# AlwinEsch/pvr.rtl.radiofm

Hardware: AMD Instinct MI355X
Metric: IQ MS/s demodulated (whole node) + achieved HBM GB/s on FIR stage (higher is better)
Workload: dtype f32

## Files before the change

### pvr.rtl.radiofm_amd/csrc/fmd_batch.hip

```cpp
#include "../../include/fmd.h"

#include <hip/hip_runtime.h>
#include <hip/hip_ext.h>

#include <algorithm>
#include <chrono>
#include <cmath>
#include <cstdio>
#include <cstdlib>
#include <cstring>
#include <deque>
#include <functional>
#include <map>
#include <memory>
#include <mutex>
#include <string>
#include <utility>
#include <vector>

#include "fmd_design.hpp"
#include "fmd_groups.hpp"
#include "fmd_kernels.hip.h"
#include "fmd_receiver.hpp"

// ... 19 lines not shown
enum Stage
{
  ST_IF_FIR = 0,
  ST_DEMOD_SERIAL,
  ST_RDS_HALFBAND,
  ST_RDS_LPF,
  ST_RDS_SERIAL,
  ST_RESAMPLE,
  ST_AUDIO_LPF,
  ST_AUDIO_TAIL,
  ST_ROLL,
  ST_COUNT
};
const char* kStageNames[ST_COUNT] = {"if_fir",      "demod_serial", "rds_halfband",
                                     "rds_lpf",     "rds_serial",   "resample",
                                     "audio_lpf",   "audio_tail",   "history_roll"};

template <typename T, bool HOST>
struct Buf
{
  T* p = nullptr;
  size_t n = 0;
  Buf() = default;
  Buf(Buf&& o) noexcept : p(std::exchange(o.p, nullptr)), n(std::exchange(o.n, 0)) {}
  ~Buf() { release(); }
  int alloc(size_t count, unsigned host_flags = hipHostMallocDefault)
  {
    release();
    const size_t bytes = std::max<size_t>(count, 1) * sizeof(T);
    void* v = nullptr;
    if ((HOST ? hipHostMalloc(&v, bytes, host_flags) : hipMalloc(&v, bytes)) != hipSuccess)
      return -1;
    p = static_cast<T*>(v);
    if (HOST)
      std::memset(v, 0, bytes);
    else if (hipMemset(v, 0, bytes) != hipSuccess)
    {
      release();
      return -1;
    }
    n = count;
    return 0;
  }
  void release()
  {
    if (p)
      (void)(HOST ? hipHostFree(p) : hipFree(p));
    p = nullptr;
    n = 0;
  }
};
template <typename T>
using DevBuf = Buf<T, false>;
template <typename T>
using HostBuf = Buf<T, true>;

struct Event
{
  hipEvent_t e = nullptr;
  Event() = default;
  Event(Event&& o) noexcept : e(std::exchange(o.e, nullptr)) {}
  ~Event() { release(); }
  hipError_t create(unsigned flags = hipEventDisableTiming)
  {
    release();
    return hipEventCreateWithFlags(&e, flags);
  }
  void release()
  {
    if (e)
      (void)hipEventDestroy(e);
    e = nullptr;
  }
  operator hipEvent_t() const { return e; }
};

template <typename... P, typename... A>
void launch(void (*kern)(P...), dim3 grid, dim3 block, unsigned lds, hipStream_t s, hipEvent_t ev_start,
            hipEvent_t ev_stop, A... args)
{
  static_assert(sizeof...(P) == sizeof...(A), "kernel argument count");
  if (ev_start)
    hipExtLaunchKernelGGL(kern, grid, block, lds, s, ev_start, ev_stop, 0u, static_cast<P>(args)...);
  else
    hipLaunchKernelGGL(kern, grid, block, lds, s, static_cast<P>(args)...);
}

}

struct fmd_batch
{
  fmd::Params params;
  fmd::Design des;
  unsigned C = 0, CP = 0;
  int device = 0;
  fmd_callbacks cb{};
  void* user = nullptr;
  std::vector<int> shifts;

  unsigned if_pos = 0;
  unsigned lut_idx = 0;
  float rs_pos = 0.0f;
  unsigned rds_lpf_g = 0;
  unsigned mf_g = 0;
  unsigned alpf_g = 0;
  int hist_sel = 0;
  uint32_t call_index = 0;

  unsigned min_samples = 0;
  int streams_sharing = 0;
  unsigned cpc = 1;
  unsigned Mmax = 0, Mstride = 0, Amax = 0, Rmax = 0;
  std::vector<unsigned> hb_nmax;
  unsigned lastM = 0, lastA = 0, lastR = 0;

  DevBuf<float2> lut, hist[2], demod[2], br[2], mix[2], rdsraw[2], rlpf[2], rs[2], alp[2];
  std::vector<DevBuf<float2>> hbbuf;
  DevBuf<float> if_coeff, rs_coeff, rds_lpf_taps, mf_taps2, audio_taps, ktab;
  DevBuf<float> rpll, rmf, tap_sync;
  DevBuf<double> sctab, sctab256;
  DevBuf<int> pidx;
  static constexpr unsigned kBrFront = 32;
  float2* brp(int q) const { return br[q].p + size_t(kBrFront) * CP; }
  unsigned rs_margin = 0, rs_row = 0;
  int rsr_R = 0, rsr_NW = 0;
  unsigned rsr_nbr = 0, rsr_nbm = 0;
  int rsr_rb = 0;
  DevBuf<float> rsr_tab;
  DevBuf<int> rsr_head, rsr_steps;
  int rsr_mode = -1;
  int n_cus = 256;
  struct HbfPlan
  {
    unsigned n_in = 0, S = 0;
    DevBuf<fmd::HbStep> steps;
    DevBuf<int> seg_first;
  };
  std::vector<std::unique_ptr<HbfPlan>> hbf_plans;
  DevBuf<float2> hbf_tail1, hbf_tail2;
  int hbf_mode = -1;
  static constexpr unsigned kOscH = 64;
  DevBuf<fmd::HbOsc> osc_tab[4];
  HostBuf<fmd::HbOsc> h_osc;
  Event osc_ev[8];
  bool osc_ev_used[8] = {};
  size_t h_osc_stride = 0;
  float osc_re = 1.0f, osc_im = 0.0f;
  bool osc_on = false;
  int dbg_nomix = 1;
  int dbg_fir_nt = 0;
  int dbg_serial_claim = 0;
  int dbg_hb4 = 1, dbg_ring4 = 1;
  int dbg_fir_ro = 2;
  int dbg_lpf_late = -1;
  double host_ms[4] = {0, 0, 0, 0};
  unsigned host_calls = 0;
  DevBuf<long long> serial_probe;
  int dbg_stage_mask = 63;
  DevBuf<float> fstate;
  DevBuf<int> istate;
  DevBuf<uint16_t> r_data;
  static constexpr int NSLOT = 8;
  static_assert(NSLOT == 8, "osc_ev / osc_ev_used above");
  DevBuf<fmd::RdsGroupRec> queue[NSLOT];
  DevBuf<unsigned> queue_counts;
  unsigned* qcount(int q) const { return queue_counts.p + q; }
  uint32_t drained_call[NSLOT] = {};
  HostBuf<unsigned> h_counts;
  HostBuf<fmd::RdsGroupRec> h_recs;
  unsigned queue_cap = 0;
  Event ev_drained[NSLOT];
  bool drained_pending[NSLOT] = {};
  static constexpr unsigned kExportCursors = 16;
  DevBuf<unsigned> export_cursor;
  unsigned export_seq = 0;
  fmd::ChannelState st{};
  std::vector<fmd::HbCoef> hbcoef;
  fmd::HbChainTaps hb_taps{};

  DevBuf<float> h_iq, h_audio;
  DevBuf<float> h_mpx;
  int dbg_mpx_timing = 0;
  Event mpx_ev[8][2];
  bool mpx_ev_used[8] = {};
  DevBuf<unsigned long long> pcm_clip;

  struct SelTable
  {
    DevBuf<int> d;
    HostBuf<int> h;
    Event read;
    hipStream_t stream = nullptr;
    bool used = false;
  };
  struct Selection
  {
    bool on = false;
    unsigned n_total = 0;
    std::vector<unsigned> list;
    std::vector<int2> ent;
    bool dirty = false;
    std::vector<std::unique_ptr<SelTable>> pool;
    int cur = -1;
  };
  Selection sel_audio, sel_mpx;
  bool decoder_owned = false;

  std::vector<std::unique_ptr<fmd::GroupDecoder>> gdec;

  int profiling = 0;
  int write_taps = 0;

  int concurrency = 1;
  hipStream_t s_fir = nullptr, s_ser = nullptr, s_post = nullptr, s_rds = nullptr, s_lpf = nullptr;
  struct LightJob
  {
    unsigned R = 0, A = 0, mf_g = 0, alpf_g = 0;
    unsigned rds_lpf_g = 0;
    const unsigned* org = nullptr;
    int q = 0, es = 0, sq = 0;
    bool events = true;
    bool lpf_here = false;
    int audio_after = -1;
    bool status_after_rds = false;
    hipEvent_t prev_aud = nullptr;
    uint32_t call_index = 0;
    void* d_audio = nullptr;
    int pcm = 0;
    size_t audio_stride = 0;
    hipEvent_t tl0 = nullptr, tl1 = nullptr;
    Selection* asel = nullptr;
  };
  std::vector<std::unique_ptr<fmd_batch>> subs;
  std::vector<unsigned> sub_ch0;
  bool owns_streams = true;
  hipEvent_t vheavy[2] = {nullptr, nullptr};
  hipEvent_t sched_prev2 = nullptr;
  bool split_post = false;
  bool serial_exclusive = false;
  enum { EV_IN, EV_FIR, EV_INDONE, EV_SER, EV_AUD, EV_RDS, EV_HEAVY, EV_RDSH, EV_ALP, EV_DEC, EV_ROLL, EV_N };
  Event cev[NSLOT][EV_N];
  uint32_t slot_call[NSLOT] = {};
  std::vector<Event> ev;
  unsigned prof_calls = 0;

  HostBuf<unsigned> h_err;
  bool failed = false;
  std::string fail_msg;
  unsigned spin_limit = 1u << 20;
  bool if_dry_run = false;
  HostBuf<unsigned> h_status;
  DevBuf<unsigned> d_status;
  unsigned host_seq = 0;

  fmd_params cparams{};
  std::unique_ptr<fmd_batch> twin;
  DevBuf<float2> twin_iq;
  DevBuf<float> twin_audio;
  std::mutex log_mu;
  std::vector<std::vector<std::pair<uint32_t, int>>> shift_log;
  std::vector<uint32_t> gdec_epoch;
  struct Edit
  {
    unsigned ch;
    int shift;
    bool reset;
    int imp = -1;
  };
  std::vector<Edit> edits;
  bool edits_pending = false;
  fmd::RestartTable restart_tab{};
  int restart_group[fmd::kRestartMaxRegions] = {};
  int restart_skip = -1;
  unsigned restart_rows_cap = 0;
  HostBuf<int2> h_edits;
  HostBuf<float2> h_rows;
  DevBuf<int2> d_edits;
  DevBuf<float2> d_rows;
  Event edit_ev[NSLOT];
  bool edit_ev_used[NSLOT] = {};
  Event edit_done;
  unsigned restart_seq = 0;
  DevBuf<unsigned> org;
  bool origins_live = false;
  int dbg_reset_keep_phase = 0;

  unsigned n_cap = 0;
  bool map_on = false, map_dirty = false;
  int capture_walk = 1;
  std::vector<unsigned> cmap;
  DevBuf<uint2> d_walk;
  HostBuf<uint2> h_walk;
  Event walk_ev[NSLOT];
  bool walk_ev_used[NSLOT] = {};

  fmd::StateTable state_tab{};
  int state_group[fmd::kStateMaxRegions] = {};
  size_t state_bytes = 0;
  int state_skip = -1;
  struct PendingImport
  {
    int slot = 0;
    unsigned n_cols = 0, n_rows = 0;
    size_t rows_at = 0, payload_at = 0, bytes = 0;
    bool origins_live = false;
    std::vector<fmd::StateEdit> list;
// ... 1366 lines not shown
}

int fmd_batch_process_device_u8(fmd_batch* b, const uint8_t* d_iq_u8, size_t iq_channel_stride,
                                unsigned samples, float* d_audio, size_t audio_channel_stride,
                                unsigned* out_floats, void* stream)
{
  return fmd_batch_process_device_fmt(b, d_iq_u8, FMD_IQ_U8, iq_channel_stride, samples, d_audio,
                                      audio_channel_stride, out_floats, stream);
}

static bool slot_eligible(const fmd_batch* b, int q, int lag)
{
  return b->slot_call[q] != 0 && b->slot_call[q] + uint32_t(lag) <= b->call_index;
}

static int wait_impl(fmd_batch* b, int lag, void* stream_, bool take_lost)
{
  if (!b || lag < 0 || lag > 4)
    return fail(FMD_ERR_ARG, "fmd_batch_wait: bad argument (lag must be 0..4)");
  hipStream_t stream = static_cast<hipStream_t>(stream_);
  HIPCHK(hipSetDevice(b->device));
  if (is_shell(b))
  {
    for (auto& sb : b->subs)
    {
      const int rc = wait_impl(sb.get(), lag, stream_, false);
      if (rc < 0)
        return check_device_errors(b);
    }
    if (int rc = check_device_errors(b))
      return rc;
    return take_lost ? take_lost_groups(b) : FMD_OK;
  }
  auto wait_if_pending = [&](hipEvent_t e) {
    if (hipEventQuery(e) == hipSuccess)
      return hipSuccess;
    (void)hipGetLastError();
    return hipStreamWaitEvent(stream, e, 0);
  };
  for (int q = 0; q < fmd_batch::NSLOT; q++)
    if (slot_eligible(b, q, lag))
    {
      HIPCHK(wait_if_pending(b->cev[q][fmd_batch::EV_AUD]));
      HIPCHK(wait_if_pending(b->cev[q][fmd_batch::EV_RDS]));
      HIPCHK(wait_if_pending(b->cev[q][fmd_batch::EV_INDONE]));
      HIPCHK(wait_if_pending(b->cev[q][fmd_batch::EV_ROLL]));
    }
  if (int rc = check_device_errors(b))
    return rc;
  return take_lost ? take_lost_groups(b) : FMD_OK;
}

int fmd_batch_wait_lagged(fmd_batch* b, int lag, void* stream_)
{
  return wait_impl(b, lag, stream_, true);
}

int fmd_batch_take_rds_lost(fmd_batch* b)
{
  if (!b)
    return fail(FMD_ERR_ARG, "null batch");
  return take_lost_groups(b) == FMD_WARN_RDS_LOST ? 1 : 0;
}

int fmd_batch_debug_set_spin_limit(fmd_batch* b, unsigned limit)
{
  if (!b)
    return fail(FMD_ERR_ARG, "null batch");
  b->spin_limit = limit;
  b->st.spin_limit = limit;
  for (auto& sb : b->subs)
    fmd_batch_debug_set_spin_limit(sb.get(), limit);
  return FMD_OK;
}

int fmd_batch_debug_restart_skip(fmd_batch* b, int region)
{
  if (!b)
    return fail(FMD_ERR_ARG, "null batch");
  if (region < -1 || region >= kRestartRegionCount)
  {
    std::string names;
    for (const char* r : kRestartRegions)
      names += std::string(names.empty() ? "" : ", ") + r;
    return fail(FMD_ERR_ARG, "fmd_batch_debug_restart_skip: -1 or the index of a region (" + names + ")");
  }
  b->restart_skip = region;
  for (auto& sb : b->subs)
    sb->restart_skip = region;
  return FMD_OK;
}

int fmd_batch_debug_reset_keep_ring_phase(fmd_batch* b, int on)
{
  if (!b)
    return fail(FMD_ERR_ARG, "null batch");
  b->dbg_reset_keep_phase = on != 0;
  for (auto& sb : b->subs)
    sb->dbg_reset_keep_phase = on != 0;
  return FMD_OK;
}

int fmd_batch_debug_host_ms(fmd_batch* b, float out[4])
{
  if (!b || !out)
    return fail(FMD_ERR_ARG, "null argument");
  const unsigned n = b->host_calls;
  for (int i = 0; i < 4; i++)
  {
    out[i] = n ? float(b->host_ms[i] / n) : 0.0f;
    b->host_ms[i] = 0.0;
  }
  b->host_calls = 0;
  return int(n);
}

int fmd_batch_debug_set(fmd_batch* b, const char* key, int value)
{
  if (!b || !key)
    return fail(FMD_ERR_ARG, "null argument");
  const std::string k(key);
  HIPCHK(hipSetDevice(b->device));
  HIPCHK(hipDeviceSynchronize());
  if (is_shell(b))
  {
    for (auto& sb : b->subs)
      if (int rc = fmd_batch_debug_set(sb.get(), key, value))
        return rc;
    return FMD_OK;
  }
  if (k == "resampler")
  {
    if (value > 0 && b->rsr_R == 0)
      return fail(FMD_ERR_ARG, "fmd_batch_debug_set: no form of k_resample_ring fits this geometry");
    b->rsr_mode = value < 0 ? -1 : (value ? 1 : 0);
  }
  else if (k == "fir_nt")
    b->dbg_fir_nt = std::max(0, value);
  else if (k == "serial_claim")
    b->dbg_serial_claim = value != 0;
  else if (k == "serial_exclusive")
    b->serial_exclusive = value != 0;
  else if (k == "split_post")
    b->split_post = value != 0;
  else if (k == "hb4")
    b->dbg_hb4 = value != 0;
  else if (k == "ring4")
    b->dbg_ring4 = value != 0;
  else if (k == "lpf_late")
    b->dbg_lpf_late = value < 0 ? -1 : std::min(value, 2);
  else if (k == "stage_mask")
    b->dbg_stage_mask = value & 63;
  else if (k == "fir_ro")
    b->dbg_fir_ro = (value == 2 || value == 3) ? value : 1;
  else if (k == "serial_probe")
  {
    HIPCHK(hipSetDevice(b->device));
    HIPCHK(hipDeviceSynchronize());
    b->serial_probe.release();
    if (value && b->serial_probe.alloc(size_t(8) * 3 * (b->CP / 64)))
      return fail(FMD_ERR_DEVICE, "serial probe allocation failed");
  }
  else if (k == "halfband_chain")
  {
    b->hbf_mode = value < 0 ? -1 : (value ? 1 : 0);
    if (value > 0 && b->call_index == 0 && b->h_osc.p && b->des.hb.size() == 3 &&
        b->des.hb[0].len - 1 <= int(fmd_batch::kOscH))
      b->osc_on = true;
  }
  else if (k == "nomix")
    b->dbg_nomix = value != 0;
  else if (k == "rsr_form")
  {
    bool ok = false;
    for (int f = std::max(0, std::min(2, value)); f < 3 && !ok; f++)
      ok = rsr_configure(b, f);
  }
  else
    return fail(FMD_ERR_ARG, "fmd_batch_debug_set: unknown key '" + k + "'");
  return FMD_OK;
}

int fmd_batch_enable_retune(fmd_batch* b)
{
  if (!b)
    return fail(FMD_ERR_ARG, "fmd_batch_enable_retune: null batch");
  if (b->twin)
    return FMD_OK;
  if (b->call_index != 0)
    return fail(FMD_ERR_STATE, "fmd_batch_enable_retune: only before the batch's first call");
  HIPCHK(hipSetDevice(b->device));
  fmd_batch* tw = nullptr;
  const int zero_shift = 0;
  if (int rc = create_one(&b->cparams, 1, &zero_shift, b->device, nullptr, nullptr, b, &tw))
    return rc;
  std::unique_ptr<fmd_batch> twin(tw);
  twin->concurrency = 2;
  if (b->twin_iq.alloc(FMD_MAX_BLOCK) || b->twin_audio.alloc(fmd_batch_max_audio_floats(tw, FMD_MAX_BLOCK)))
    return fail(FMD_ERR_DEVICE, "fmd_batch_enable_retune: device allocation failed");
  if (is_shell(b))
  {
    for (auto& sb : b->subs)
      if (int rc = build_restart_table(sb.get(), tw))
        return rc;
  }
  else if (int rc = build_restart_table(b, tw))
    return rc;
  HIPCHK(hipDeviceSynchronize());
  {
    std::lock_guard<std::mutex> lk(b->log_mu);
    b->shift_log.resize(b->C);
  }
  b->gdec_epoch.resize(b->C, 0u);
  b->twin = std::move(twin);
  return FMD_OK;
}

int fmd_batch_retune_channels(fmd_batch* b, const unsigned* channels, const int* shifts, unsigned n)
{
  if (!b || !channels || !shifts)
    return fail(FMD_ERR_ARG, "fmd_batch_retune_channels: null argument");
  if (b->failed)
    return fail(FMD_ERR_ARG, "fmd_batch_retune_channels: the batch has failed (fmd_batch_reset clears it)");
  if (!b->twin)
    return fail(FMD_ERR_STATE, "fmd_batch_retune_channels: retuning is not enabled (fmd_batch_enable_retune)");
  if (int rc = check_channel_list(b, channels, nullptr, n, "fmd_batch_retune_channels"))
    return rc;
  const uint32_t k = b->call_index + 1;
  std::lock_guard<std::mutex> lk(b->log_mu);
  for (unsigned i = 0; i < n; i++)
  {
    unsigned lc = 0;
    fmd_batch* ob = owner_of(b, channels[i], &lc);
    ob->edits.push_back(fmd_batch::Edit{lc, shifts[i], false});
    drop_gdec_import(b, channels[i], k);
    auto& log = b->shift_log[channels[i]];
    if (!log.empty() && log.back().first == k)
      log.back().second = shifts[i];
    else
      log.emplace_back(k, shifts[i]);
  }
  b->edits_pending = true;
  return FMD_OK;
}

int fmd_batch_reset_channels(fmd_batch* b, const unsigned* channels, unsigned n)
{
  if (!b || !channels)
    return fail(FMD_ERR_ARG, "fmd_batch_reset_channels: null argument");
  if (b->failed)
    return fail(FMD_ERR_ARG, "fmd_batch_reset_channels: the batch has failed (fmd_batch_reset clears it)");
  std::vector<unsigned> seen(channels, channels + n);
  std::sort(seen.begin(), seen.end());
  if (n && seen.back() >= b->C)
    return fail(FMD_ERR_ARG, "fmd_batch_reset_channels: channel " + std::to_string(seen.back()) + " out of range");
  if (std::adjacent_find(seen.begin(), seen.end()) != seen.end())
    return fail(FMD_ERR_ARG, "fmd_batch_reset_channels: a channel is listed twice");
  if (n == 0)
    return FMD_OK;
  const uint32_t k = b->call_index + 1;
  std::lock_guard<std::mutex> lk(b->log_mu);
  if (b->shift_log.empty())
  {
    b->shift_log.resize(b->C);
    b->gdec_epoch.assign(b->C, 0u);
  }
  for (unsigned i = 0; i < n; i++)
  {
    unsigned lc = 0;
    fmd_batch* ob = owner_of(b, channels[i], &lc);
    ob->edits.push_back(fmd_batch::Edit{lc, 0, true});
    drop_gdec_import(b, channels[i], k);
    auto& log = b->shift_log[channels[i]];
    if (log.empty() || log.back().first != k)
      log.emplace_back(k, log.empty() ? b->shifts[channels[i]] : log.back().second);
  }
  b->edits_pending = true;
  return FMD_OK;
}

int fmd_batch_wait(fmd_batch* b, void* stream_)
{
  return fmd_batch_wait_lagged(b, 0, stream_);
}

int fmd_batch_set_channels_per_capture(fmd_batch* b, unsigned channels_per_capture)
{
  if (!b)
    return fail(FMD_ERR_ARG, "null batch");
  const unsigned k = channels_per_capture ? channels_per_capture : 1u;
  if (b->C % k)
    return fail(FMD_ERR_ARG, "fmd_batch_set_channels_per_capture: the channel count is not a multiple of it");
  for (size_t i = 0; i < b->subs.size(); i++)
    if (b->sub_ch0[i] % k || b->subs[i]->C % k)
      return fail(FMD_ERR_ARG, "fmd_batch_set_channels_per_capture: with " + std::to_string(b->C) +
                                   " channels the batch runs as sub-batches of " + std::to_string(b->subs[0]->C) +
                                   ", which is not a multiple of it");
  HIPCHK(hipSetDevice(b->device));
  HIPCHK(hipDeviceSynchronize());
  b->cpc = k;
  for (auto& sb : b->subs)
    sb->cpc = k;
  b->map_on = false;
  b->n_cap = 0;
  for (auto& sb : b->subs)
  {
    sb->map_on = false;
// ... 1201 lines not shown
```

### pvr.rtl.radiofm_amd/csrc/fmd_batch_if.inc.hpp

```cpp
namespace
{

template <class IN>
using FirFn = void (*)(const typename IN::elem*, size_t, unsigned, const float2*, float2*, const float2*,
                       unsigned, unsigned, const float*, unsigned, unsigned, unsigned, unsigned, float2*,
                       unsigned, unsigned, unsigned, unsigned, const uint2*);

template <class IN, int TILE, int E, bool MAP, bool RB128 = false>
int launch_if_stage_t(fmd_batch* b, const void* d_iq, size_t iq_channel_stride, unsigned N, unsigned pos,
                      unsigned M, int q, hipStream_t sF, const std::function<void(int)>& mark,
                      hipEvent_t ev_start, hipEvent_t ev_stop)
{
  const fmd::Design& d = b->des;
  const unsigned C = b->C, D = d.D, T = d.table_size;
  const unsigned ntiles = (M + TILE - 1) / TILE;
  const size_t region = ((size_t(TILE - 1) * D + d.if_order + 2u * (1u << E) + 2u) >> E) + 2u;
  const bool longasm = TILE == 256 && d.if_order >= 512;
  const size_t lds = (region << E) * sizeof(float2) + (longasm ? 32 * sizeof(float2) : 0);
  if (lds > 160 * 1024)
    return fail(FMD_ERR_ARG, "IF filter window does not fit in LDS");
  const bool pow2 = (T & (T - 1)) == 0 && T <= 2u * TILE && (size_t(TILE) * D) % T == 0;
  const unsigned rounds = unsigned(((size_t(TILE - 1) * D + d.if_order + 2) / 2 + TILE - 1) / TILE);
  FirFn<IN> kfn = &fmd::k_if_fir<IN, TILE, 1, false, E, false, false, false, MAP>;
  if (pow2)
    kfn = rounds <= 2 ? &fmd::k_if_fir<IN, TILE, 2, true, E, false, false, false, MAP>
        : rounds <= 4 ? &fmd::k_if_fir<IN, TILE, 4, true, E, false, false, false, MAP>
        : rounds <= 6 ? &fmd::k_if_fir<IN, TILE, 6, true, E, false, false, false, MAP>
        : rounds <= 7 ? &fmd::k_if_fir<IN, TILE, 7, true, E, false, false, false, MAP>
                      : &fmd::k_if_fir<IN, TILE, 8, true, E, false, false, false, MAP>;
  if (pow2 && longasm)
    kfn = &fmd::k_if_fir<IN, TILE, 8, true, E, TILE == 256 && (E == 0 || RB128), false,
                         TILE == 256 && RB128 && (E >= 1), MAP>;
  const bool shfl = b->params.fir_reduction == 1 && TILE == 64 && E == 0 && pow2 && rounds <= 8;
  if (shfl)
    kfn = &fmd::k_if_fir<IN, TILE, 8, true, E, false, TILE == 64 && E == 0, false, MAP>;
  const bool fma = b->params.fir_reduction == 2;
  const int fir_nt = fma ? 2 : b->dbg_fir_nt ? b->dbg_fir_nt : (b->concurrency == 2 && b->serial_exclusive ? 2 : 1);
  unsigned nblocks = C * ntiles, ntiles_l = ntiles;
  size_t lds_l = lds;
  FirFn<IN> kfn3 = nullptr;
  if (TILE == 64 && E == 0 && pow2 && rounds == 7 && fir_nt > 1 && !shfl)
  {
    const unsigned nt = fir_nt >= 8 ? 8u : fir_nt >= 4 ? 4u : fir_nt == 3 ? 3u : 2u;
    kfn = nt == 8 ? &fmd::k_if_fir_mt<IN, 7, 8, MAP>
        : nt == 4 ? &fmd::k_if_fir_mt<IN, 7, 4, MAP>
        : nt == 3 ? &fmd::k_if_fir_mt<IN, 7, 3, MAP>
                  : &fmd::k_if_fir_mt<IN, 7, 2, MAP>;
    nblocks = C * ((ntiles + nt - 1) / nt);
    const unsigned RO = fma ? 2u : unsigned(b->dbg_fir_ro), T3 = 64 * RO;
    const unsigned rounds3 = unsigned(((size_t(T3 - 1) * D + d.if_order + 2) / 2 + 63) / 64);
    if (RO > 1 && nt == 2 && d.if_order == 88 && D == 11 && (size_t(T3) * D) % T == 0 &&
        rounds3 <= (RO == 3 ? 18u : 12u))
    {
      kfn3 = RO == 3 ? &fmd::k_if_fir_mt3<IN, 18, 2, 3, 88, 11, false, MAP>
             : fma   ? &fmd::k_if_fir_mt3<IN, 12, 2, 2, 88, 11, true, MAP>
                     : &fmd::k_if_fir_mt3<IN, 12, 2, 2, 88, 11, false, MAP>;
      ntiles_l = (M + T3 - 1) / T3;
      lds_l = (size_t(T3 - 1) * D + d.if_order + 4) * sizeof(float2);
      nblocks = C * ((ntiles_l + 1) / 2);
    }
  }
  if (fma && !kfn3)
    return fail(FMD_ERR_ARG, "FMD_FIR_FMA_PARITY_WAIVED: the fused multiply-add form exists for the reference geometry "
                             "only (88-tap IF filter, downsample 11, power-of-two tuner table)");
  if (b->if_dry_run)
    return FMD_OK;
  if (lds > 64 * 1024)
    (void)hipFuncSetAttribute(reinterpret_cast<const void*>(kfn),
                              hipFuncAttributeMaxDynamicSharedMemorySize, 160 * 1024);
  const typename IN::elem* x = static_cast<const typename IN::elem*>(d_iq);
  mark(0);
  launch(kfn3 ? kfn3 : kfn, dim3(nblocks), dim3(TILE), unsigned(lds_l), sF, ev_start, ev_stop, x, iq_channel_stride,
         N, b->hist[b->hist_sel].p, b->hist[b->hist_sel ^ 1].p, b->lut.p, T, b->lut_idx, b->if_coeff.p, d.if_order, D,
         pos, M, b->demod[q].p, b->Mstride, ntiles_l, (C % 8 == 0) ? 1u : 0u, b->cpc,
         MAP ? (const uint2*)b->d_walk.p : nullptr);
  mark(1);
  hipLaunchKernelGGL((fmd::k_if_level<IN, MAP>), dim3(C), dim3(64), 0, sF, x, iq_channel_stride, N, b->lut.p, T,
                     b->lut_idx, b->st, b->cpc, MAP ? (const uint2*)b->d_walk.p : nullptr);
  return FMD_OK;
}

template <class IN, int TILE, bool MAP>
int launch_if_stage_e(fmd_batch* b, const void* d_iq, size_t iq_channel_stride, unsigned N, unsigned pos,
                      unsigned M, int q, hipStream_t sF, const std::function<void(int)>& mark,
                      hipEvent_t ev_start, hipEvent_t ev_stop)
{
  const unsigned D = b->des.D;
  if (D % 2 != 0)
    return launch_if_stage_t<IN, TILE, 0, MAP>(b, d_iq, iq_channel_stride, N, pos, M, q, sF, mark, ev_start, ev_stop);
  if (D % 4 != 0)
  {
    const unsigned T = b->des.table_size;
    const bool pow2 = (T & (T - 1)) == 0 && T <= 2u * TILE && (size_t(TILE) * D) % T == 0;
    if (TILE == 256 && b->des.if_order >= 512 && pow2)
      return launch_if_stage_t<IN, TILE, 0, MAP>(b, d_iq, iq_channel_stride, N, pos, M, q, sF, mark, ev_start, ev_stop);
    return launch_if_stage_t<IN, TILE, 1, MAP>(b, d_iq, iq_channel_stride, N, pos, M, q, sF, mark, ev_start, ev_stop);
  }
  {
    const unsigned T = b->des.table_size;
    const bool pow2 = (T & (T - 1)) == 0 && T <= 2u * TILE && (size_t(TILE) * D) % T == 0;
    if (TILE == 256 && b->des.if_order >= 512 && pow2)
    {
      if (D % 8 != 0)
        return launch_if_stage_t<IN, TILE, 1, MAP, true>(b, d_iq, iq_channel_stride, N, pos, M, q, sF, mark, ev_start,
                                                    ev_stop);
      return launch_if_stage_t<IN, TILE, 2, MAP, true>(b, d_iq, iq_channel_stride, N, pos, M, q, sF, mark, ev_start,
                                                  ev_stop);
    }
  }
  return launch_if_stage_t<IN, TILE, 2, MAP>(b, d_iq, iq_channel_stride, N, pos, M, q, sF, mark, ev_start, ev_stop);
}

template <class IN, bool MAP>
int launch_if_stage_m(fmd_batch* b, const void* d_iq, size_t iq_channel_stride, unsigned N, unsigned pos,
                      unsigned M, int q, hipStream_t sF, const std::function<void(int)>& mark,
                      hipEvent_t ev_start, hipEvent_t ev_stop)
{
  const fmd::Design& d = b->des;
  const unsigned T = d.table_size;
  auto fits = [&](unsigned tile) {
    const bool pow2 = (T & (T - 1)) == 0 && T <= 2u * tile && (size_t(tile) * d.D) % T == 0;
    const size_t lds = (size_t(tile - 1) * d.D + d.if_order + 4) * sizeof(float2);
    return pow2 && d.if_order <= 4u * tile * d.D / 8u && lds <= 16 * 1024;
  };
  if (fits(64))
    return launch_if_stage_e<IN, 64, MAP>(b, d_iq, iq_channel_stride, N, pos, M, q, sF, mark, ev_start, ev_stop);
  if (fits(128))
    return launch_if_stage_e<IN, 128, MAP>(b, d_iq, iq_channel_stride, N, pos, M, q, sF, mark, ev_start, ev_stop);
  return launch_if_stage_e<IN, 256, MAP>(b, d_iq, iq_channel_stride, N, pos, M, q, sF, mark, ev_start, ev_stop);
}

template <class IN>
int launch_if_stage(fmd_batch* b, const void* d_iq, size_t iq_channel_stride, unsigned N, unsigned pos,
                    unsigned M, int q, hipStream_t sF, const std::function<void(int)>& mark,
                    hipEvent_t ev_start, hipEvent_t ev_stop)
{
  if (b->map_on)
    return launch_if_stage_m<IN, true>(b, d_iq, iq_channel_stride, N, pos, M, q, sF, mark, ev_start, ev_stop);
  return launch_if_stage_m<IN, false>(b, d_iq, iq_channel_stride, N, pos, M, q, sF, mark, ev_start, ev_stop);
}

}
```

### pvr.rtl.radiofm_amd/csrc/fmd_k_common.hip.h

```cpp
#pragma once

#include <hip/hip_runtime.h>
#include <stdint.h>

#include "fmd_math.h"

namespace fmd
{
struct DemodConsts
{
  float pll_alpha, pll_beta, nco_hl, nco_ll, demod_gain;
  float p_minfreq, p_maxfreq, p_b0, p_a1, p_a2, p_lf_b0, p_lf_b1, p_minsignal;
  int p_lock_delay;
  float osc_cos, osc_sin;
};

struct RdsConsts
{
  float pll_alpha, pll_beta, nco_hl, nco_ll;
  float bs_b0, bs_b1, bs_b2, bs_a1, bs_a2;
  int mf_taps;
};

struct AudioConsts
{
  float de_alpha;
  float n_b0, n_b1, n_b2, n_a1, n_a2;
};

enum FSlot
{
  F_NCO_PHASE, F_NCO_INCR, F_DC_OFF,
  F_IF_LEVEL, F_BB_MEAN, F_BB_LEVEL,
  F_P_I1, F_P_I2, F_P_Q1, F_P_Q2, F_P_X1, F_P_FREQ, F_P_PHASE, F_P_LEVEL,
  F_OSC_RE, F_OSC_IM,
  F_R_PHASE, F_R_FREQ, F_R_W1, F_R_W2, F_R_LAST_SYNC, F_R_LAST_SLOPE, F_R_LAST_DATA,
  F_DE_RE, F_DE_IM, F_N_W1A, F_N_W2A, F_N_W1B, F_N_W2B,
  F_AUDIO_MEAN, F_AUDIO_RMS, F_AUDIO_LEVEL,
  F_SLOTS
};
enum ISlot
{
  I_P_LOCK_CNT, I_STEREO,
  I_STEREO_Q0, I_STEREO_Q1, I_STEREO_Q2, I_STEREO_Q3,
  I_R_LAST_BIT, I_R_BITS, I_R_BLOCK, I_R_BITPOS, I_R_STATE, I_R_BOFF,
  I_R_ERRORS, I_R_SEQ, I_SLOTS
};
enum DevErr : unsigned
{
  DEVERR_SERIAL_HANDSHAKE = 1u,
  DEVERR_RDS_QUEUE_FULL = 1u
};
enum HostStatusWord
{
  HS_SEQ_BEGIN, HS_IF_LEVEL, HS_BB_MEAN, HS_BB_LEVEL, HS_P_LEVEL, HS_STEREO, HS_R_STATE,
  HS_AUDIO_MEAN, HS_AUDIO_RMS, HS_AUDIO_LEVEL, HS_SEQ_END, HS_WORDS
};
struct ChannelState
{
  float* f;
  int* i;
  uint16_t* r_data;
  unsigned* err;
  unsigned* hs;
  unsigned* ds;
  unsigned spin_limit;
  unsigned CP;
  __host__ __device__ float* F(int slot) const { return f + (size_t)slot * CP; }
  __host__ __device__ int* I(int slot) const { return i + (size_t)slot * CP; }
};

struct RdsGroupRec
{
  uint32_t channel;
  uint32_t call_index;
  uint32_t seq;
  uint16_t blocks[4];
};

__device__ __forceinline__ void wave_prio(unsigned p)
{
  if (p == 1u)
    __builtin_amdgcn_s_setprio(1);
  else if (p == 2u)
    __builtin_amdgcn_s_setprio(2);
  else if (p == 3u)
    __builtin_amdgcn_s_setprio(3);
}
__device__ __forceinline__ void lds_barrier()
{
  asm volatile("s_waitcnt lgkmcnt(0)\n\ts_barrier" ::: "memory");
}
__device__ __forceinline__ void lds_wave_sync()
{
  asm volatile("s_waitcnt lgkmcnt(0)" ::: "memory");
}

__device__ __forceinline__ void lds_publish(unsigned lds_addr, unsigned value)
{
  asm volatile("ds_write_b32 %0, %1" ::"v"(lds_addr), "v"(value) : "memory");
}
__device__ __forceinline__ void dev_error(unsigned* err, unsigned bit)
{
  __hip_atomic_fetch_or(err, bit, __ATOMIC_RELAXED, __HIP_MEMORY_SCOPE_SYSTEM);
}
__device__ __forceinline__ void lds_wait_ge(unsigned lds_addr, unsigned value, unsigned limit, unsigned* err)
{
  bool ok = false;
#pragma unroll 1
  for (unsigned spins = 0; spins < limit; spins++)
  {
    unsigned seen;
    asm volatile("ds_read_b32 %0, %1\n\ts_waitcnt lgkmcnt(0)" : "=v"(seen) : "v"(lds_addr) : "memory");
    if ((unsigned)__builtin_amdgcn_readfirstlane((int)seen) >= value)
    {
      ok = true;
      break;
    }
    __builtin_amdgcn_s_sleep(1);
  }
  if (!ok && __builtin_amdgcn_readfirstlane((int)threadIdx.x) == (int)threadIdx.x)
    dev_error(err, DEVERR_SERIAL_HANDSHAKE);
}

__device__ __forceinline__ unsigned capture_of(unsigned c, unsigned cpc)
{
  return cpc > 1u ? (unsigned)__builtin_amdgcn_readfirstlane((int)(c / cpc)) : c;
}

__device__ __forceinline__ unsigned walk_take(const uint2* __restrict__ walk, unsigned& c)
{
  const uint2 w = walk[c];
  c = w.x;
  return w.y;
}

__device__ __forceinline__ float2 cmul(float2 a, float2 b)
{
  return make_float2(a.x * b.x - a.y * b.y, a.x * b.y + a.y * b.x);
}

typedef float fmd_f2v __attribute__((ext_vector_type(2)));

}
```

### pvr.rtl.radiofm_amd/csrc/fmd_k_if.hip.h

```cpp
#pragma once

#include "fmd_k_common.hip.h"

namespace fmd
{

__device__ __forceinline__ void fir_long_odd_asm(fmd_f2v& acc2, unsigned& a0, unsigned klo, unsigned khi,
                                                 unsigned& cnt)
{
  asm volatile(
      "s_mov_b32 s72, %3\n\t"
      "s_mov_b32 s73, %4\n\t"
      "s_load_dwordx16 s[40:55], s[72:73], 0x0\n\t"
      "ds_read2_b64 v[64:67], %1 offset0:15 offset1:14\n\t"
      "ds_read2_b64 v[68:71], %1 offset0:13 offset1:12\n\t"
      "ds_read2_b64 v[72:75], %1 offset0:11 offset1:10\n\t"
      "ds_read2_b64 v[76:79], %1 offset0:9 offset1:8\n\t"
      "ds_read2_b64 v[80:83], %1 offset0:7 offset1:6\n\t"
      "ds_read2_b64 v[84:87], %1 offset0:5 offset1:4\n\t"
      "ds_read2_b64 v[88:91], %1 offset0:3 offset1:2\n\t"
      "ds_read2_b64 v[92:95], %1 offset0:1\n\t"
      "v_subrev_u32 %1, 128, %1\n\t"
      "s_add_u32 s72, s72, 64\n\t"
      "s_addc_u32 s73, s73, 0\n\t"
// ... 850 lines not shown
}

template <class IN, int UNROLL, int NT, bool MAP = false>
__global__ __launch_bounds__(64) void k_if_fir_mt(const typename IN::elem* __restrict__ iq,
                                                  size_t chan_stride, unsigned N,
                                                  const float2* __restrict__ hist_in,
                                                  float2* __restrict__ hist_out,
                                                  const float2* __restrict__ lut, unsigned T,
                                                  unsigned lut_idx0, const float* __restrict__ coeff,
                                                  unsigned order, unsigned D, unsigned pos, unsigned M,
                                                  float2* __restrict__ out, unsigned Mstride,
                                                  unsigned ntiles, unsigned xcd_map, unsigned cpc,
                                                 const uint2* __restrict__ walk)
{
  typedef typename IN::pair pair_t;
  constexpr int TILE = 64;
  extern __shared__ __attribute__((aligned(16))) float2 win[];
  __builtin_amdgcn_s_setprio(1);
  const unsigned ngroups = (ntiles + NT - 1) / NT;
  unsigned c, tg;
  if (xcd_map)
  {
    const unsigned xcd = blockIdx.x & 7u, slot = blockIdx.x >> 3;
    c = (slot / ngroups) * 8u + xcd;
    tg = slot % ngroups;
  }
  else
  {
    c = blockIdx.x / ngroups;
    tg = blockIdx.x % ngroups;
  }
  const unsigned tid = threadIdx.x;
  unsigned cap;
  if constexpr (MAP)
    cap = walk_take(walk, c);
  else
    cap = capture_of(c, cpc);
  const typename IN::elem* __restrict__ x = iq + (size_t)cap * chan_stride;
  const float2* __restrict__ l = lut + (size_t)c * T;
  const unsigned mask = T - 1;
  const int kfull_all = (int)(N & ~1u);
  float2 l0, l1;
  {
    const int k_al0 = ((int)(pos + tg * NT * TILE * D) - (int)order) & ~1;
    const unsigned li = (lut_idx0 + (unsigned)k_al0 + 2u * tid) & mask;
    l0 = l[li];
    l1 = l[(li + 1) & mask];
  }
  pair_t v[UNROLL];
  auto issue = [&](unsigned tile) {
    const unsigned m0 = tile * TILE;
    const unsigned nout = min((unsigned)TILE, M - m0);
    const int p_first = (int)(pos + m0 * D);
    const int k_lo = p_first - (int)order;
    const int k_hi = p_first + (int)((nout - 1) * D);
    const int k_al = k_lo & ~1;
    const int kfull = min(k_hi, kfull_all);
    const int ifirst = k_al < 0 ? (-k_al) >> 1 : 0;
    const int npairs = (kfull - k_al + 1) >> 1;
    const pair_t* __restrict__ src = reinterpret_cast<const pair_t*>(x) + (k_al >> 1);
#pragma unroll
    for (int u = 0; u < UNROLL; u++)
      v[u] = src[max(min(u * TILE + (int)tid, npairs - 1), ifirst)];
  };
  const unsigned t_first = tg * NT;
  issue(t_first);
  for (unsigned i = 0; i < (unsigned)NT; i++)
  {
    const unsigned tile = t_first + i;
    if (tile >= ntiles)
      break;
    const unsigned m0 = tile * TILE;
    const unsigned nout = min((unsigned)TILE, M - m0);
    const int p_first = (int)(pos + m0 * D);
    const int k_lo = p_first - (int)order;
    const int k_hi = p_first + (int)((nout - 1) * D);
    const int k_al = k_lo & ~1;
    if (k_lo < 0)
    {
      const float2* __restrict__ h = hist_in + (size_t)c * order;
      const int nh = min(-k_lo, k_hi - k_lo);
      for (int q = (int)tid; q < nh; q += TILE)
        win[q + (k_lo - k_al)] = h[(int)order + k_lo + q];
    }
    {
      const int kfull = min(k_hi, kfull_all);
      const int ifirst = k_al < 0 ? (-k_al) >> 1 : 0;
      const int npairs = (kfull - k_al + 1) >> 1;
      float4* dst = reinterpret_cast<float4*>(win);
#pragma unroll
      for (int u = 0; u < UNROLL; u++)
      {
        const int q = u * TILE + (int)tid;
        if (q >= ifirst && q < npairs)
        {
          float2 a, b;
          IN::unpack(v[u], a, b);
          a = cmul(a, l0);
          b = cmul(b, l1);
          dst[q] = make_float4(a.x, a.y, b.x, b.y);
        }
      }
      const pair_t* __restrict__ src = reinterpret_cast<const pair_t*>(x) + (k_al >> 1);
      for (int q = UNROLL * TILE + (int)tid; q < npairs; q += TILE)
      {
        float2 a, b;
        IN::unpack(src[max(q, ifirst)], a, b);
        a = cmul(a, l0);
        b = cmul(b, l1);
        if (q >= ifirst)
          dst[q] = make_float4(a.x, a.y, b.x, b.y);
      }
      for (int k = max(kfull, 0) + (int)tid; k < k_hi; k += TILE)
        win[k - k_al] = cmul(IN::one(x, k), l[(lut_idx0 + (unsigned)k) & mask]);
    }
    lds_wave_sync();
    if (i + 1 < (unsigned)NT && tile + 1 < ntiles)
      issue(tile + 1);
    if (tid < nout)
    {
      float2 acc = make_float2(0.0f, 0.0f);
      const float2* w = win + (k_lo - k_al) + tid * D + order;
#pragma unroll 8
      for (unsigned j = 1; j <= order; j++)
      {
        const float k = coeff[j];
        const float2 sm = w[-(int)j];
        acc.x += sm.x * k;
        acc.y += sm.y * k;
      }
      out[(size_t)c * Mstride + m0 + tid] = acc;
    }
    if (tile == ntiles - 1)
    {
      float2* __restrict__ ho = hist_out + (size_t)c * order;
      const float2* __restrict__ hi = hist_in + (size_t)c * order;
      const unsigned keep = N < order ? order - N : 0u;
      for (unsigned q = tid; q < order; q += TILE)
      {
        if (q < keep)
          ho[q] = hi[q + N];
        else
        {
          const unsigned k = N + q - order;
          ho[q] = cmul(IN::one(x, k), l[(lut_idx0 + k) % T]);
        }
      }
    }
    lds_wave_sync();
  }
}

template <class IN, int UNROLL, int NT, int RO = 3, int ORD = 88, int DEC = 11, bool FMA = false, bool MAP = false>
__global__ __launch_bounds__(64) void k_if_fir_mt3(const typename IN::elem* __restrict__ iq,
                                                   size_t chan_stride, unsigned N,
                                                   const float2* __restrict__ hist_in,
                                                   float2* __restrict__ hist_out,
                                                   const float2* __restrict__ lut, unsigned T,
                                                   unsigned lut_idx0, const float* __restrict__ coeff,
                                                   unsigned order, unsigned D, unsigned pos, unsigned M,
                                                   float2* __restrict__ out, unsigned Mstride,
                                                   unsigned ntiles, unsigned xcd_map, unsigned cpc,
                                                 const uint2* __restrict__ walk)
{
  typedef typename IN::pair pair_t;
  static_assert(RO == 2 || RO == 3, "outputs per lane (lane stride RO D samples: conflict-free for 3)");
  constexpr int LANES = 64, TILE = LANES * RO;
  extern __shared__ __attribute__((aligned(16))) float2 win[];
  __builtin_amdgcn_s_setprio(1);
  const unsigned ngroups = (ntiles + NT - 1) / NT;
  unsigned c, tg;
  if (xcd_map)
  {
    const unsigned xcd = blockIdx.x & 7u, slot = blockIdx.x >> 3;
    c = (slot / ngroups) * 8u + xcd;
    tg = slot % ngroups;
  }
  else
  {
    c = blockIdx.x / ngroups;
    tg = blockIdx.x % ngroups;
  }
  const unsigned tid = threadIdx.x;
  unsigned cap;
  if constexpr (MAP)
    cap = walk_take(walk, c);
  else
    cap = capture_of(c, cpc);
  const typename IN::elem* __restrict__ x = iq + (size_t)cap * chan_stride;
  const float2* __restrict__ l = lut + (size_t)c * T;
  const unsigned mask = T - 1;
  const int kfull_all = (int)(N & ~1u);
  float2 l0, l1;
  {
    const int k_al0 = ((int)(pos + tg * NT * TILE * D) - (int)order) & ~1;
    const unsigned li = (lut_idx0 + (unsigned)k_al0 + 2u * tid) & mask;
    l0 = l[li];
    l1 = l[(li + 1) & mask];
  }
  pair_t v[UNROLL];
  auto issue = [&](unsigned tile) {
    const unsigned m0 = tile * TILE;
    const unsigned nout = min((unsigned)TILE, M - m0);
    const int p_first = (int)(pos + m0 * D);
    const int k_lo = p_first - (int)order;
    const int k_hi = p_first + (int)((nout - 1) * D);
    const int k_al = k_lo & ~1;
    const int kfull = min(k_hi, kfull_all);
    const int ifirst = k_al < 0 ? (-k_al) >> 1 : 0;
    const int npairs = (kfull - k_al + 1) >> 1;
    const pair_t* __restrict__ src = reinterpret_cast<const pair_t*>(x) + (k_al >> 1);
#pragma unroll
    for (int u = 0; u < UNROLL; u++)
      v[u] = src[max(min(u * LANES + (int)tid, npairs - 1), ifirst)];
  };
  const unsigned t_first = tg * NT;
  issue(t_first);
  for (unsigned i = 0; i < (unsigned)NT; i++)
  {
    const unsigned tile = t_first + i;
    if (tile >= ntiles)
      break;
    const unsigned m0 = tile * TILE;
    const unsigned nout = min((unsigned)TILE, M - m0);
    const int p_first = (int)(pos + m0 * D);
    const int k_lo = p_first - (int)order;
    const int k_hi = p_first + (int)((nout - 1) * D);
    const int k_al = k_lo & ~1;
    if (k_lo < 0)
    {
      const float2* __restrict__ h = hist_in + (size_t)c * order;
      const int nh = min(-k_lo, k_hi - k_lo);
      for (int q = (int)tid; q < nh; q += LANES)
        win[q + (k_lo - k_al)] = h[(int)order + k_lo + q];
    }
    {
      const int kfull = min(k_hi, kfull_all);
      const int ifirst = k_al < 0 ? (-k_al) >> 1 : 0;
      const int npairs = (kfull - k_al + 1) >> 1;
      float4* dst = reinterpret_cast<float4*>(win);
#pragma unroll
      for (int u = 0; u < UNROLL; u++)
      {
        const int q = u * LANES + (int)tid;
        if (q >= ifirst && q < npairs)
        {
          float2 a, b;
          IN::unpack(v[u], a, b);
          a = cmul(a, l0);
          b = cmul(b, l1);
          dst[q] = make_float4(a.x, a.y, b.x, b.y);
        }
      }
      const pair_t* __restrict__ src = reinterpret_cast<const pair_t*>(x) + (k_al >> 1);
      for (int q = UNROLL * LANES + (int)tid; q < npairs; q += LANES)
      {
        float2 a, b;
        IN::unpack(src[max(q, ifirst)], a, b);
        a = cmul(a, l0);
        b = cmul(b, l1);
        if (q >= ifirst)
          dst[q] = make_float4(a.x, a.y, b.x, b.y);
      }
      for (int k = max(kfull, 0) + (int)tid; k < k_hi; k += LANES)
        win[k - k_al] = cmul(IN::one(x, k), l[(lut_idx0 + (unsigned)k) & mask]);
    }
    lds_wave_sync();
    if (i + 1 < (unsigned)NT && tile + 1 < ntiles)
      issue(tile + 1);
    if (tid * RO < nout)
    {
      static_assert(ORD % DEC == 0 && ORD >= RO * DEC, "stretches of DEC samples");
      constexpr int NB = ORD / DEC, NS = NB + (RO - 1);
      float2 acc[RO];
#pragma unroll
      for (int r = 0; r < RO; r++)
        acc[r] = make_float2(0.0f, 0.0f);
      const float2* w = win + (k_lo - k_al) + (tid * RO + (RO - 1)) * DEC + ORD;
      auto stretch = [&](int st, auto all) {
        const float2* ws = w - st * DEC;
#pragma unroll
        for (int i = 1; i <= DEC; i++)
        {
          const float2 sm = ws[-i];
#pragma unroll
          for (int r = 0; r < RO; r++)
          {
            const int sb = st - (RO - 1 - r);
            if (decltype(all)::value || (sb >= 0 && sb < NB))
            {
              const float cj = coeff[sb * DEC + i];
              if (FMA)
              {
                const fmd_f2v t = __builtin_elementwise_fma(fmd_f2v{sm.x, sm.y}, fmd_f2v{cj, cj},
                                                            fmd_f2v{acc[r].x, acc[r].y});
                acc[r] = make_float2(t.x, t.y);
              }
              else
              {
                acc[r].x += sm.x * cj;
                acc[r].y += sm.y * cj;
              }
            }
          }
        }
      };
#pragma unroll
      for (int st = 0; st < RO - 1; st++)
        stretch(st, std::false_type{});
#pragma unroll 1
      for (int st = RO - 1; st < NB; st++)
        stretch(st, std::true_type{});
#pragma unroll
      for (int st = NB; st < NS; st++)
        stretch(st, std::false_type{});
      float2* __restrict__ op = out + (size_t)c * Mstride + m0 + tid * RO;
#pragma unroll
      for (int r = 0; r < RO; r++)
        if (tid * RO + r < nout)
          op[r] = acc[r];
    }
    if (tile == ntiles - 1)
    {
      float2* __restrict__ ho = hist_out + (size_t)c * order;
      const float2* __restrict__ hi = hist_in + (size_t)c * order;
      const unsigned keep = N < order ? order - N : 0u;
      for (unsigned q = tid; q < order; q += LANES)
      {
        if (q < keep)
          ho[q] = hi[q + N];
        else
        {
          const unsigned k = N + q - order;
          ho[q] = cmul(IN::one(x, k), l[(lut_idx0 + k) % T]);
        }
      }
    }
    lds_wave_sync();
  }
}

template <class IN, bool MAP = false>
__global__ __launch_bounds__(64) void k_if_level(const typename IN::elem* __restrict__ iq,
                                                 size_t chan_stride, unsigned N,
                                                 const float2* __restrict__ lut, unsigned T,
                                                 unsigned lut_idx0, ChannelState st, unsigned cpc,
                                                 const uint2* __restrict__ walk)
{
  __shared__ float term[1024];
  unsigned c = blockIdx.x;
  const unsigned n = (N + 63) / 64;
  unsigned cap;
  if constexpr (MAP)
    cap = walk_take(walk, c);
  else
    cap = capture_of(c, cpc);
  const typename IN::elem* __restrict__ x = iq + (size_t)cap * chan_stride;
  const float2* __restrict__ l = lut + (size_t)c * T;
  for (unsigned i = threadIdx.x; i < n; i += 64)
  {
    const float2 s = cmul(IN::one(x, i), l[(lut_idx0 + i) % T]);
    term[i] = s.x * s.x + s.y * s.y;
  }
  __syncthreads();
  if (threadIdx.x == 0)
  {
    float level = 0.0f;
    for (unsigned i = 0; i < n; ++i)
      level += term[i];
    const float rms = sqrtf(level / (float)n);
    st.F(F_IF_LEVEL)[c] = 0.95f * st.F(F_IF_LEVEL)[c] + 0.05f * rms;
  }
}

}
```

Before: 299,400.

## Add bounds-free interior-tile fast path to the 2-output IF FIR kernel

Splits each workgroup's two tiles into interior and boundary kinds at compile time. Interior tiles skip history loads, clamped indices and tail handling, and stage the window with unconditional vector loads and a packed complex multiply (v_pk_mul/v_pk_add). The change also scalarizes the channel base pointer via readfirstlane, sets waves_per_eu occupancy hints, and rounds LDS up to a fixed size. A new negative fir_ro setting disables the interior path. The cost is more template instantiations, code size and register pressure.

```diff
diff --git a/pvr.rtl.radiofm_amd/csrc/fmd_batch.hip b/pvr.rtl.radiofm_amd/csrc/fmd_batch.hip
--- a/pvr.rtl.radiofm_amd/csrc/fmd_batch.hip
+++ b/pvr.rtl.radiofm_amd/csrc/fmd_batch.hip
@@ -195,6 +195,7 @@
   int dbg_serial_claim = 0;
   int dbg_hb4 = 1, dbg_ring4 = 1;
   int dbg_fir_ro = 2;
+  bool dbg_fir_interior = true;
   int dbg_lpf_late = -1;
   double host_ms[4] = {0, 0, 0, 0};
   unsigned host_calls = 0;
@@ -1867,7 +1868,11 @@
   else if (k == "stage_mask")
     b->dbg_stage_mask = value & 63;
   else if (k == "fir_ro")
-    b->dbg_fir_ro = (value == 2 || value == 3) ? value : 1;
+  {
+    const int ro = value < 0 ? -value : value;
+    b->dbg_fir_ro = (ro == 2 || ro == 3) ? ro : 1;
+    b->dbg_fir_interior = value >= 0;
+  }
   else if (k == "serial_probe")
   {
     HIPCHK(hipSetDevice(b->device));
diff --git a/pvr.rtl.radiofm_amd/csrc/fmd_batch_if.inc.hpp b/pvr.rtl.radiofm_amd/csrc/fmd_batch_if.inc.hpp
--- a/pvr.rtl.radiofm_amd/csrc/fmd_batch_if.inc.hpp
+++ b/pvr.rtl.radiofm_amd/csrc/fmd_batch_if.inc.hpp
@@ -56,7 +56,8 @@
              : fma   ? &fmd::k_if_fir_mt3<IN, 12, 2, 2, 88, 11, true, MAP>
                      : &fmd::k_if_fir_mt3<IN, 12, 2, 2, 88, 11, false, MAP>;
       ntiles_l = (M + T3 - 1) / T3;
-      lds_l = (size_t(T3 - 1) * D + d.if_order + 4) * sizeof(float2);
+      lds_l = RO == 2 ? size_t(12) * 64 * 2 * sizeof(float2) : (size_t(T3 - 1) * D + d.if_order + 4) * sizeof(float2);
+      static_assert(size_t(12) * 64 * 2 >= size_t(127) * 11 + 88 + 4, "the rounds' pairs hold the window");
       nblocks = C * ((ntiles_l + 1) / 2);
     }
   }
@@ -72,7 +73,8 @@
   mark(0);
   launch(kfn3 ? kfn3 : kfn, dim3(nblocks), dim3(TILE), unsigned(lds_l), sF, ev_start, ev_stop, x, iq_channel_stride,
          N, b->hist[b->hist_sel].p, b->hist[b->hist_sel ^ 1].p, b->lut.p, T, b->lut_idx, b->if_coeff.p, d.if_order, D,
-         pos, M, b->demod[q].p, b->Mstride, ntiles_l, (C % 8 == 0) ? 1u : 0u, b->cpc,
+         pos, M, b->demod[q].p, b->Mstride, ntiles_l,
+         ((C % 8 == 0) ? 1u : 0u) | ((kfn3 && !b->dbg_fir_interior) ? 2u : 0u), b->cpc,
          MAP ? (const uint2*)b->d_walk.p : nullptr);
   mark(1);
   hipLaunchKernelGGL((fmd::k_if_level<IN, MAP>), dim3(C), dim3(64), 0, sF, x, iq_channel_stride, N, b->lut.p, T,
diff --git a/pvr.rtl.radiofm_amd/csrc/fmd_k_common.hip.h b/pvr.rtl.radiofm_amd/csrc/fmd_k_common.hip.h
--- a/pvr.rtl.radiofm_amd/csrc/fmd_k_common.hip.h
+++ b/pvr.rtl.radiofm_amd/csrc/fmd_k_common.hip.h
@@ -135,11 +135,27 @@
   return w.y;
 }
 
+__device__ __forceinline__ size_t uniform_u64(size_t a)
+{
+  const unsigned lo = (unsigned)__builtin_amdgcn_readfirstlane((int)(unsigned)a);
+  const unsigned hi = (unsigned)__builtin_amdgcn_readfirstlane((int)(unsigned)(a >> 32));
+  return ((size_t)hi << 32) | lo;
+}
+
 __device__ __forceinline__ float2 cmul(float2 a, float2 b)
 {
   return make_float2(a.x * b.x - a.y * b.y, a.x * b.y + a.y * b.x);
 }
 
+__device__ __forceinline__ float2 cmul_pk(float2 a, float2 l)
+{
+  float2 p, q, r;
+  asm("v_pk_mul_f32 %0, %1, %2 op_sel_hi:[0,1]" : "=v"(p) : "v"(a), "v"(l));
+  asm("v_pk_mul_f32 %0, %1, %2 op_sel:[1,1] op_sel_hi:[1,0]" : "=v"(q) : "v"(a), "v"(l));
+  asm("v_pk_add_f32 %0, %1, %2 neg_lo:[0,1]" : "=v"(r) : "v"(p), "v"(q));
+  return r;
+}
+
 typedef float fmd_f2v __attribute__((ext_vector_type(2)));
 
 }
diff --git a/pvr.rtl.radiofm_amd/csrc/fmd_k_if.hip.h b/pvr.rtl.radiofm_amd/csrc/fmd_k_if.hip.h
--- a/pvr.rtl.radiofm_amd/csrc/fmd_k_if.hip.h
+++ b/pvr.rtl.radiofm_amd/csrc/fmd_k_if.hip.h
@@ -1026,7 +1026,8 @@
 }
 
 template <class IN, int UNROLL, int NT, int RO = 3, int ORD = 88, int DEC = 11, bool FMA = false, bool MAP = false>
-__global__ __launch_bounds__(64) void k_if_fir_mt3(const typename IN::elem* __restrict__ iq,
+__global__ __launch_bounds__(64) __attribute__((amdgpu_waves_per_eu(RO == 2 ? 4 : 3)))
+void k_if_fir_mt3(const typename IN::elem* __restrict__ iq,
                                                    size_t chan_stride, unsigned N,
                                                    const float2* __restrict__ hist_in,
                                                    float2* __restrict__ hist_out,
@@ -1044,7 +1045,7 @@
   __builtin_amdgcn_s_setprio(1);
   const unsigned ngroups = (ntiles + NT - 1) / NT;
   unsigned c, tg;
-  if (xcd_map)
+  if (xcd_map & 1u)
   {
     const unsigned xcd = blockIdx.x & 7u, slot = blockIdx.x >> 3;
     c = (slot / ngroups) * 8u + xcd;
@@ -1061,7 +1062,7 @@
     cap = walk_take(walk, c);
   else
     cap = capture_of(c, cpc);
-  const typename IN::elem* __restrict__ x = iq + (size_t)cap * chan_stride;
+  const typename IN::elem* __restrict__ x = iq + uniform_u64((size_t)cap * chan_stride);
   const float2* __restrict__ l = lut + (size_t)c * T;
   const unsigned mask = T - 1;
   const int kfull_all = (int)(N & ~1u);
@@ -1088,27 +1089,63 @@
     for (int u = 0; u < UNROLL; u++)
       v[u] = src[max(min(u * LANES + (int)tid, npairs - 1), ifirst)];
   };
-  const unsigned t_first = tg * NT;
-  issue(t_first);
-  for (unsigned i = 0; i < (unsigned)NT; i++)
-  {
-    const unsigned tile = t_first + i;
-    if (tile >= ntiles)
-      break;
+  constexpr bool HAS_INTERIOR = RO == 2;
+  constexpr int LDSP = RO == 2 ? UNROLL * LANES : ((TILE - 1) * DEC + ORD + 4) / 2;
+  static_assert((LDSP + LANES - 1) / LANES == UNROLL, "the rounds stage one window");
+  auto interior = [&](unsigned tile) {
+    const unsigned m0 = tile * TILE;
+    const int k_lo = (int)(pos + m0 * D) - (int)order;
+    return HAS_INTERIOR && !(xcd_map & 2u) && m0 + TILE <= M && k_lo >= 0 && (k_lo & ~1) + 2 * UNROLL * LANES <= kfull_all;
+  };
+  auto issue_interior = [&](unsigned tile) {
+    const int k_al = ((int)(pos + tile * TILE * D) - (int)order) & ~1;
+    const pair_t* __restrict__ src = reinterpret_cast<const pair_t*>(x) + (k_al >> 1);
+#pragma unroll
+    for (int u = 0; u < UNROLL; u++)
+      v[u] = src[u * LANES + (int)tid];
+  };
+  auto run_tile = [&](unsigned tile, auto interior_c, auto next_c, auto first_c) {
+    constexpr bool INTERIOR = decltype(interior_c)::value;
+    constexpr int NEXT = decltype(next_c)::value;
+    if (decltype(first_c)::value)
+    {
+      if (INTERIOR)
+        issue_interior(tile);
+      else
+        issue(tile);
+    }
     const unsigned m0 = tile * TILE;
     const unsigned nout = min((unsigned)TILE, M - m0);
     const int p_first = (int)(pos + m0 * D);
     const int k_lo = p_first - (int)order;
     const int k_hi = p_first + (int)((nout - 1) * D);
     const int k_al = k_lo & ~1;
-    if (k_lo < 0)
+    if (INTERIOR)
     {
-      const float2* __restrict__ h = hist_in + (size_t)c * order;
-      const int nh = min(-k_lo, k_hi - k_lo);
-      for (int q = (int)tid; q < nh; q += LANES)
-        win[q + (k_lo - k_al)] = h[(int)order + k_lo + q];
+      float4* dst = reinterpret_cast<float4*>(win);
+#pragma unroll
+      for (int u = 0; u < UNROLL; u++)
+      {
+        const int q = u * LANES + (int)tid;
+        if ((u + 1) * LANES <= LDSP || q < LDSP)
+        {
+          float2 a, b;
+          IN::unpack(v[u], a, b);
+          a = cmul_pk(a, l0);
+          b = cmul_pk(b, l1);
+          dst[q] = make_float4(a.x, a.y, b.x, b.y);
+        }
+      }
     }
+    else
     {
+      if (k_lo < 0)
+      {
+        const float2* __restrict__ h = hist_in + (size_t)c * order;
+        const int nh = min(-k_lo, k_hi - k_lo);
+        for (int q = (int)tid; q < nh; q += LANES)
+          win[q + (k_lo - k_al)] = h[(int)order + k_lo + q];
+      }
       const int kfull = min(k_hi, kfull_all);
       const int ifirst = k_al < 0 ? (-k_al) >> 1 : 0;
       const int npairs = (kfull - k_al + 1) >> 1;
@@ -1140,7 +1177,9 @@
         win[k - k_al] = cmul(IN::one(x, k), l[(lut_idx0 + (unsigned)k) & mask]);
     }
     lds_wave_sync();
-    if (i + 1 < (unsigned)NT && tile + 1 < ntiles)
+    if (NEXT == 2)
+      issue_interior(tile + 1);
+    else if (NEXT == 1)
       issue(tile + 1);
     if (tid * RO < nout)
     {
@@ -1211,6 +1250,40 @@
       }
     }
     lds_wave_sync();
+  };
+  static_assert(NT == 2, "the kinds of a workgroup's two tiles are told apart below");
+  typedef std::true_type Y;
+  typedef std::false_type F;
+  typedef std::integral_constant<int, 0> N0;
+  typedef std::integral_constant<int, 1> N1;
+  typedef std::integral_constant<int, 2> N2;
+  const unsigned t0 = tg * NT;
+  const bool has1 = t0 + 1 < ntiles;
+  const bool in0 = has1 && interior(t0), in1 = has1 && interior(t0 + 1);
+  if (HAS_INTERIOR && in0)
+  {
+    if (in1)
+      run_tile(t0, Y{}, N2{}, Y{});
+    else
+      run_tile(t0, Y{}, N0{}, Y{});
+  }
+  else
+  {
+    if (HAS_INTERIOR && in1)
+      run_tile(t0, F{}, N2{}, Y{});
+    else if (has1)
+      run_tile(t0, F{}, N1{}, Y{});
+    else
+      run_tile(t0, F{}, N0{}, Y{});
+  }
+  if (HAS_INTERIOR && in1)
+    run_tile(t0 + 1, Y{}, N0{}, F{});
+  else if (has1)
+  {
+    if (HAS_INTERIOR && in0)
+      run_tile(t0 + 1, F{}, N0{}, Y{});
+    else
+      run_tile(t0 + 1, F{}, N0{}, F{});
   }
 }
 
```

Result: faster. 302,700 (median of 6 runs) (+1.1%).
